# YuliangXiu/ICON

Measured on NVIDIA H100. Metric: M query-points/sec at 256^3 grid, higher is better.
Workload: dtype f32

## Files before the change

### icon_b200/csrc/common.cuh

```cuda
#pragma once
#include <cuda_runtime.h>
#include <stdint.h>
#include <stdio.h>

#include "../../include/icon_b200.h"

namespace icon {

void set_error(const char *fmt, ...);
void count_launch(int n = 1);

#define ICON_CHECK_ARG(cond, ...)                 \
    do {                                          \
        if (!(cond)) {                            \
            icon::set_error(__VA_ARGS__);         \
            return ICON_EINVAL;                   \
        }                                         \
    } while (0)

#define ICON_CUDA(expr)                                                              \
    do {                                                                             \
        cudaError_t _e = (expr);                                                     \
        if (_e != cudaSuccess) {                                                     \
            icon::set_error("%s:%d %s -> %s", __FILE__, __LINE__, #expr,             \
// ... 20 lines not shown
    return true;
}
int device_sm_count();

bool pdl_enabled();
#ifdef __CUDACC__
__device__ __forceinline__ void pdl_launch_dependents() { asm volatile("griddepcontrol.launch_dependents;" ::: "memory"); }
__device__ __forceinline__ void pdl_wait() { asm volatile("griddepcontrol.wait;" ::: "memory"); }
template <typename... KArgs, typename... Args>
static inline cudaError_t launch_pdl(void (*kernel)(KArgs...), dim3 grid, dim3 block, size_t smem, cudaStream_t stream,
                                     Args &&...args) {
    cudaLaunchConfig_t cfg = {};
    cfg.gridDim = grid; cfg.blockDim = block; cfg.dynamicSmemBytes = smem; cfg.stream = stream;
    cudaLaunchAttribute attr[1];
    attr[0].id = cudaLaunchAttributeProgrammaticStreamSerialization;
    attr[0].val.programmaticStreamSerializationAllowed = 1;
    cfg.attrs = attr; cfg.numAttrs = pdl_enabled() ? 1 : 0;
    return cudaLaunchKernelEx(&cfg, kernel, KArgs(args)...);
}

__device__ __forceinline__ void stats_add3(double *w, double s) {
    const double a = trunc(s), r = s - a;
    const double b = rint(r * 4294967296.0) * (1.0 / 4294967296.0);
    const double c = rint((r - b) * 18446744073709551616.0) * (1.0 / 18446744073709551616.0);
    if (a != 0.0) atomicAdd(w, a);
    if (b != 0.0) atomicAdd(w + 1, b);
    if (c != 0.0) atomicAdd(w + 2, c);
}
__device__ __forceinline__ void stats_add(double *st, double s1, double s2) { stats_add3(st, s1); stats_add3(st + 3, s2); }
__device__ __forceinline__ double stats_sum(const double *st) { return st[0] + (st[1] + st[2]); }
__device__ __forceinline__ double stats_sumsq(const double *st) { return st[3] + (st[4] + st[5]); }
#endif

struct Carver {
    char *base;
    size_t off;
    explicit Carver(void *p) : base((char *)p), off(0) {}
    template <typename T>
    T *take(size_t n) {
        off = align_up(off, 256);
        T *r = (T *)(base ? base + off : nullptr);
        off += n * sizeof(T);
        return r;
    }
    size_t total() const { return align_up(off, 256); }
};

constexpr int TREE_MAX_LEVELS = 17;
constexpr int RAY_GRID = 256;
constexpr int RAY_LIST_PER_FACE = 64;

constexpr int BRICK_AX = 32;
constexpr int NBRICK = BRICK_AX * BRICK_AX * BRICK_AX;
constexpr int BRICK_MAX_LEAVES = 4096;
constexpr int64_t BRICK_LIST_CAP = 1 << 24;
static inline int64_t brick_list_cap(int F) {
    const int64_t all = (int64_t)NBRICK * ((F + 3) / 4);
    return all < BRICK_LIST_CAP ? all : BRICK_LIST_CAP;
}

struct MeshHeader {
    float y0, z0, inv_cy, inv_cz;
    int ray_overflow;
    int brick_built;
    int brick_overflow;
    int pad;
};

struct FaceTree {
    float4 *tri_s;
    float4 *sph_s;
    int32_t *order;
    float4 *nodes;
    int F;
    int nlevels;
    int lvl_cnt[TREE_MAX_LEVELS];
    int lvl_off[TREE_MAX_LEVELS];
};

struct MeshView : FaceTree {
    const float4 *tri;
    const float4 *sph;
    const float4 *attr;
    const float4 *rbox;
    float *vnormals;
    unsigned long long *keys;
    int32_t *rcount;
    int32_t *roff;
    int32_t *rlist;
    MeshHeader *hdr;
    void *scan_ws;
    float4 *bxyz;
    int32_t *bperm;
    float *brec;
    int32_t *bface;
    float *bub;
    int32_t *boff;
    unsigned short *blist;
    int64_t brick_cap;
    int V;
};
size_t mesh_ws_bytes(int V, int F);
MeshView mesh_view(const void *ws, int V, int F);
void bricks_forget(const MeshView &m);

void profile_mark(int i, cudaStream_t stream);

size_t scan_ws_bytes(int64_t n);
int scan_exclusive_i32(const int32_t *in, int32_t *out, int64_t n, int64_t *d_total ,
                       void *ws, cudaStream_t stream);

}
```

### icon_b200/csrc/face_tree.cuh

```cuda
#pragma once
#include <float.h>

#include "common.cuh"
#include "geom.cuh"

namespace icon {

__device__ __forceinline__ float box_dist2(V3 p, float4 lo, float4 hi) {
    const float dx = fmaxf(fmaxf(lo.x - p.x, p.x - hi.x), 0.f);
    const float dy = fmaxf(fmaxf(lo.y - p.y, p.y - hi.y), 0.f);
    const float dz = fmaxf(fmaxf(lo.z - p.z, p.z - hi.z), 0.f);
    return fmaf(dz, dz, fmaf(dy, dy, dx * dx));
}
__device__ __forceinline__ float box_far2(V3 p, float4 lo, float4 hi) {
    const float dx = fmaxf(fabsf(lo.x - p.x), fabsf(hi.x - p.x));
    const float dy = fmaxf(fabsf(lo.y - p.y), fabsf(hi.y - p.y));
    const float dz = fmaxf(fabsf(lo.z - p.z), fabsf(hi.z - p.z));
    return fmaf(dz, dz, fmaf(dy, dy, dx * dx));
}
__device__ __forceinline__ float warp_max(float v) {
    for (int o = 16; o; o >>= 1) v = fmaxf(v, __shfl_xor_sync(0xffffffffu, v, o));
    return v;
}
__device__ __forceinline__ float warp_min(float v) {
// ... 38 lines not shown
    tri[2] = make_float4(ac.z, 0.f, 0.f, 0.f);
    *sph = make_float4(sc.x, sc.y, sc.z, sr);
    return sc;
}

__device__ __forceinline__ void write_leaf_box(const FaceTree &t, int n) {
    float4 lo = make_float4(FLT_MAX, FLT_MAX, FLT_MAX, 0.f), hi = make_float4(-FLT_MAX, -FLT_MAX, -FLT_MAX, 0.f);
    for (int k = 4 * n; k < min(4 * n + 4, t.F); ++k) {
        const Tri tr = load_tri(t.tri_s + 3 * (size_t)k);
        const V3 vs[3] = {tr.a, mk3(tr.a.x + tr.ab.x, tr.a.y + tr.ab.y, tr.a.z + tr.ab.z),
                          mk3(tr.a.x + tr.ac.x, tr.a.y + tr.ac.y, tr.a.z + tr.ac.z)};
        for (int j = 0; j < 3; ++j) {
            lo.x = fminf(lo.x, vs[j].x); hi.x = fmaxf(hi.x, vs[j].x);
            lo.y = fminf(lo.y, vs[j].y); hi.y = fmaxf(hi.y, vs[j].y);
            lo.z = fminf(lo.z, vs[j].z); hi.z = fmaxf(hi.z, vs[j].z);
        }
    }
    t.nodes[2 * (size_t)n] = lo;
    t.nodes[2 * (size_t)n + 1] = hi;
}

__device__ __forceinline__ void write_parent_box(const FaceTree &t, int l, int n) {
    const float4 *child = t.nodes + 2 * (size_t)t.lvl_off[l - 1];
    float4 lo = make_float4(FLT_MAX, FLT_MAX, FLT_MAX, 0.f), hi = make_float4(-FLT_MAX, -FLT_MAX, -FLT_MAX, 0.f);
    for (int c = 4 * n; c < min(4 * n + 4, t.lvl_cnt[l - 1]); ++c) {
        const float4 a = child[2 * (size_t)c], b = child[2 * (size_t)c + 1];
        lo.x = fminf(lo.x, a.x); lo.y = fminf(lo.y, a.y); lo.z = fminf(lo.z, a.z);
        hi.x = fmaxf(hi.x, b.x); hi.y = fmaxf(hi.y, b.y); hi.z = fmaxf(hi.z, b.z);
    }
    t.nodes[2 * ((size_t)t.lvl_off[l] + n)] = lo;
    t.nodes[2 * ((size_t)t.lvl_off[l] + n) + 1] = hi;
}

struct ChunkSmem {
    float4 sph[32];
    float4 tri[32][3];
    int kk[32];
};
template <typename Id, int CAP>
struct WalkSmem : ChunkSmem {
    Id fr[2][CAP];
};

template <int PPW>
struct NearestFace {
    static constexpr int REP = 32 / PPW;
    const int lane;
    V3 p;
    float tol, tol_sup;
    float best = FLT_MAX;
    int bi = 0x7fffffff;
    float sb = 0.f, ub = 0.f;
    int staged = 0;

    __device__ __forceinline__ NearestFace(V3 p_, float tol_, float tol_sup_)
        : lane(threadIdx.x & 31), p(p_), tol(tol_), tol_sup(tol_sup_) {}

    __device__ __forceinline__ float sphere_bound(float d) const {
        const float b = d * rsqrtf(d) * 1.00001f + tol;
        return d > 0.f ? b : tol;
    }

    __device__ __forceinline__ void try_face(const float4 *rec, int f) {
        const Tri tr = load_tri(rec);
        const float d = tri_sqdist(p, tr.a, tr.ab, tr.ac);
        if (d < best || (d == best && f < bi)) { best = d; bi = f; }
    }

    __device__ __forceinline__ void descend(const FaceTree &t, V3 c) {
        int node = 0;
        for (int lvl = t.nlevels - 1; lvl > 0; --lvl) {
            const int ch = 4 * node + (lane & 3);
            float a = FLT_MAX;
            int ai = ch;
            if (ch < t.lvl_cnt[lvl - 1]) {
                const float4 *nb = t.nodes + 2 * ((size_t)t.lvl_off[lvl - 1] + ch);
                a = box_dist2(c, __ldg(nb), __ldg(nb + 1));
            }
            for (int o = 1; o <= 2; o <<= 1) {
                const float ob = __shfl_xor_sync(0xffffffffu, a, o);
                const int oi = __shfl_xor_sync(0xffffffffu, ai, o);
                if (ob < a || (ob == a && oi < ai)) { a = ob; ai = oi; }
            }
            node = __shfl_sync(0xffffffffu, ai, 0);
        }
        for (int k = 4 * node; k < min(4 * node + 4, t.F); ++k) try_face(t.tri_s + 3 * (size_t)k, __ldg(t.order + k));
    }

    __device__ __forceinline__ void start_scan(float ubw) {
        sb = sphere_bound(best);
        ub = ubw * 1.00001f + tol;
    }

    __device__ __forceinline__ void test(const FaceTree &t, int k, float4 s, const float4 *tr) {
        const float dx = p.x - s.x, dy = p.y - s.y, dz = p.z - s.z;
        const float dd = fmaf(dz, dz, fmaf(dy, dy, dx * dx));
        const float l = sb + s.w;
        if (dd > l * l) return;
        const float4 r0 = tr[0], r1 = tr[1], r2 = tr[2];
        const V3 ab = mk3(r0.w, r1.x, r1.y), ac = mk3(r1.z, r1.w, r2.x);
        const float S1 = fmaf(dz, ab.z, fmaf(dy, ab.y, dx * ab.x));
        const float T1 = fmaf(dz, ac.z, fmaf(dy, ac.y, dx * ac.x));
        const float M = fmaxf(fmaxf(-(S1 + T1), fmaf(2.f, S1, -T1)), fmaf(2.f, T1, -S1)) * (1.f / 3.f);
        const float g = dd - M - tol_sup;
        if (g > 0.f && g * g > best * dd * 1.0001f) return;
        const float d = tri_sqdist(p, mk3(r0.x, r0.y, r0.z), ab, ac);
        if (!(d <= best)) return;
        const int f = __ldg(t.order + k);
        if (d < best || f < bi) { best = d; bi = f; sb = sphere_bound(d); }
    }

    __device__ __forceinline__ void merge() {
#pragma unroll
        for (int o = PPW; o < 32; o <<= 1) {
            const float ob = __shfl_xor_sync(0xffffffffu, best, o);
            const int oi = __shfl_xor_sync(0xffffffffu, bi, o);
            if (ob < best || (ob == best && oi < bi)) { best = ob; bi = oi; }
        }
    }

    __device__ __forceinline__ void chunk(const FaceTree &t, ChunkSmem &S, int leaf, float4 wlo, float4 whi) {
        bool pass = false;
        int k = 0;
        float4 s = make_float4(0.f, 0.f, 0.f, 0.f);
        if (leaf >= 0) {
            k = 4 * leaf + (lane & 3);
            if (k < t.F) {
                s = __ldg(t.sph_s + k);
                const float l2 = ub + s.w;
                pass = box_dist2(mk3(s.x, s.y, s.z), wlo, whi) <= l2 * l2;
            }
        }
        const unsigned mask = __ballot_sync(0xffffffffu, pass);
        const int cnt = __popc(mask);
        staged += cnt;
        if (pass) {
            const int at = __popc(mask & ((1u << lane) - 1u));
            const float4 *tp = t.tri_s + 3 * (size_t)k;
            S.sph[at] = s;
            S.kk[at] = k;
            S.tri[at][0] = __ldg(tp); S.tri[at][1] = __ldg(tp + 1); S.tri[at][2] = __ldg(tp + 2);
        }
        __syncwarp();
        for (int j = lane / PPW; j < cnt; j += REP) test(t, S.kk[j], S.sph[j], &S.tri[j][0]);
        if (REP > 1) {
            merge();
            sb = sphere_bound(best);
        }
        ub = fminf(ub, warp_max(sb));
        __syncwarp();
    }

    template <typename Id>
    __device__ __forceinline__ void scan_leaves(const FaceTree &t, ChunkSmem &S, const Id *leaves, int n, float4 wlo,
                                                float4 whi) {
        for (int base = 0; base < n; base += 8) {
            const int slot = base + (lane >> 2);
            chunk(t, S, slot < n ? (int)leaves[slot] : -1, wlo, whi);
// ... 68 lines not shown
```

### icon_b200/csrc/sdf.cu

```cuda
#include <float.h>

#include <algorithm>
#include <mutex>
#include <type_traits>
#include <unordered_set>

#include "common.cuh"
#include "face_tree.cuh"
#include "geom.cuh"

namespace icon {

struct Calib {
    float r[9];
    float t[3];
};

__device__ __forceinline__ V3 load_point(const float *__restrict__ pts, int64_t sc, int64_t sn,
                                         int64_t i, const Calib &cb) {
    float px = pts[i * sn], py = pts[sc + i * sn], pz = pts[2 * sc + i * sn];
    V3 o;
    o.x = fmaf(cb.r[2], pz, fmaf(cb.r[1], py, cb.r[0] * px)) + cb.t[0];
    o.y = fmaf(cb.r[5], pz, fmaf(cb.r[4], py, cb.r[3] * px)) + cb.t[1];
    o.z = fmaf(cb.r[8], pz, fmaf(cb.r[7], py, cb.r[6] * px)) + cb.t[2];
// ... 41 lines not shown
__device__ __forceinline__ unsigned spread7(unsigned v) {
    v = (v | (v << 16)) & 0x030000FFu;
    v = (v | (v << 8)) & 0x0300F00Fu;
    v = (v | (v << 4)) & 0x030C30C3u;
    v = (v | (v << 2)) & 0x09249249u;
    return v;
}

__device__ __forceinline__ int bin_of(V3 p) {
    const bool inside = p.x >= -1.f && p.x <= 1.f && p.y >= -1.f && p.y <= 1.f && p.z >= -1.f && p.z <= 1.f;
    if (!inside) return NBIN;
    const unsigned bx = min(NBIN_AX - 1, (int)((p.x + 1.f) * (NBIN_AX * 0.5f)));
    const unsigned by = min(NBIN_AX - 1, (int)((p.y + 1.f) * (NBIN_AX * 0.5f)));
    const unsigned bz = min(NBIN_AX - 1, (int)((p.z + 1.f) * (NBIN_AX * 0.5f)));
    return (int)(spread7(bx) | (spread7(by) << 1) | (spread7(bz) << 2));
}

__global__ void k_points_bin(const float *__restrict__ pts, int64_t sc, int64_t sn, int64_t N, Calib cb,
                             float4 *__restrict__ xyz4, int32_t *__restrict__ bid, int32_t *__restrict__ count) {
    const int64_t i = (int64_t)blockIdx.x * blockDim.x + threadIdx.x;
    const bool live = i < N;
    int b = -1;
    if (live) {
        const V3 p = load_point(pts, sc, sn, i, cb);
        const float in_cube = (p.x > -1.f && p.x < 1.f && p.y > -1.f && p.y < 1.f && p.z > -1.f && p.z < 1.f) ? 1.f : 0.f;
        xyz4[i] = make_float4(p.x, p.y, p.z, in_cube);
        b = bin_of(p);
        bid[i] = b;
    }
    const unsigned act = __ballot_sync(0xffffffffu, live);
    if (live) {
        const unsigned peers = __match_any_sync(act, b);
        if ((int)(threadIdx.x & 31) == __ffs(peers) - 1) atomicAdd(&count[b], __popc(peers));
    }
}

__global__ void k_points_scatter(const int32_t *__restrict__ bid, int64_t N, const int32_t *__restrict__ offset,
                                 int32_t *__restrict__ cursor, int32_t *__restrict__ perm) {
    const int64_t i = (int64_t)blockIdx.x * blockDim.x + threadIdx.x;
    const bool live = i < N;
    const int b = live ? bid[i] : -1;
    const unsigned act = __ballot_sync(0xffffffffu, live);
    if (live) {
        const unsigned peers = __match_any_sync(act, b);
        const int lane = threadIdx.x & 31, leader = __ffs(peers) - 1;
        int base = 0;
        if (lane == leader) base = atomicAdd(&cursor[b], __popc(peers));
        base = __shfl_sync(peers, base, leader);
        perm[offset[b] + base + __popc(peers & ((1u << lane) - 1u))] = (int32_t)i;
    }
}

#ifdef ICON_SDF_STATS
__device__ unsigned long long g_stats[8];
#define STAT(i, v) do { if (lane == 0) atomicAdd(&g_stats[i], (unsigned long long)(v)); } while (0)
#else
#define STAT(i, v) do { } while (0)
#endif

template <int PPW, bool BRICK>
using SdfSmem = typename std::conditional<BRICK, ChunkSmem, WalkSmem<unsigned short, fr_cap(PPW)>>::type;
template <int PPW, bool BRICK>
constexpr size_t sdf_smem_bytes() { return sizeof(SdfSmem<PPW, BRICK>) * (SW_T / 32); }

constexpr float BRICK_W = 2.0f / BRICK_AX;
constexpr float BRICK_HALF_DIAG = 0.0541266f;

__device__ __forceinline__ void brick_box(int b, float4 &lo, float4 &hi) {
    const int bx = b % BRICK_AX, by = (b / BRICK_AX) % BRICK_AX, bz = b / (BRICK_AX * BRICK_AX);
    lo = make_float4(-1.f + bx * BRICK_W, -1.f + by * BRICK_W, -1.f + bz * BRICK_W, 0.f);
    hi = make_float4(-1.f + (bx + 1) * BRICK_W, -1.f + (by + 1) * BRICK_W, -1.f + (bz + 1) * BRICK_W, 0.f);
}

__device__ __forceinline__ float leaf_key(const MeshView &m, int l, float4 lo, float4 hi) {
    const float4 a = __ldg(m.nodes + 2 * (size_t)l), z = __ldg(m.nodes + 2 * (size_t)l + 1);
    const float gx = fmaxf(fmaxf(a.x - hi.x, lo.x - z.x), 0.f);
    const float gy = fmaxf(fmaxf(a.y - hi.y, lo.y - z.y), 0.f);
    const float gz = fmaxf(fmaxf(a.z - hi.z, lo.z - z.z), 0.f);
    return fmaf(gz, gz, fmaf(gy, gy, gx * gx));
}

template <int PPW, bool BRICK>
__device__ __forceinline__ void sdf_warp(int64_t wid, SdfSmem<PPW, BRICK> &S, const float4 *__restrict__ xyz4,
                                         const int32_t *__restrict__ perm, int64_t N, const MeshView &m,
                                         float *__restrict__ rec, int32_t *__restrict__ face,
                                         int32_t *__restrict__ defer, int32_t *__restrict__ ndefer) {
    constexpr int REP = 32 / PPW;
    const int lane = threadIdx.x & 31;
    const int sub = lane % PPW, rep_id = lane / PPW;
    const int64_t pos0 = wid * PPW;
    const int64_t pos = pos0 + sub;
    if (pos0 >= N) return;
    const bool live = pos < N;
    const int64_t idx = perm[live ? pos : pos0];
    const float4 q = xyz4[idx];
    const V3 p = mk3(q.x, q.y, q.z);
    const V3 c = mk3(0.5f * (warp_min(p.x) + warp_max(p.x)), 0.5f * (warp_min(p.y) + warp_max(p.y)),
                     0.5f * (warp_min(p.z) + warp_max(p.z)));
    const float rw = warp_max(sqrtf(dot3(sub3(p, c), sub3(p, c)))) * 1.00001f + 1e-6f;
    const float4 wlo = make_float4(warp_min(p.x) - 1e-6f, warp_min(p.y) - 1e-6f, warp_min(p.z) - 1e-6f, 0.f);
    const float4 whi = make_float4(warp_max(p.x) + 1e-6f, warp_max(p.y) + 1e-6f, warp_max(p.z) + 1e-6f, 0.f);
    const MeshHeader h = *m.hdr;

    NearestFace<PPW> nf(p, 1e-6f, 1e-7f);
    if constexpr (BRICK) {
        bool ok = h.brick_built && !h.brick_overflow && c.x >= -1.f && c.x < 1.f && c.y >= -1.f && c.y < 1.f &&
                  c.z >= -1.f && c.z < 1.f;
        int b = 0;
        float4 blo, bhi;
        if (ok) {
            const int bx = min(BRICK_AX - 1, (int)((c.x + 1.f) * (BRICK_AX * 0.5f)));
            const int by = min(BRICK_AX - 1, (int)((c.y + 1.f) * (BRICK_AX * 0.5f)));
            const int bz = min(BRICK_AX - 1, (int)((c.z + 1.f) * (BRICK_AX * 0.5f)));
            b = (bz * BRICK_AX + by) * BRICK_AX + bx;
            brick_box(b, blo, bhi);
            ok = wlo.x >= blo.x && wlo.y >= blo.y && wlo.z >= blo.z && whi.x <= bhi.x && whi.y <= bhi.y && whi.z <= bhi.z;
        }
        if (!ok) {
            if (lane == 0) defer[atomicAdd(ndefer, 1)] = (int32_t)wid;
            return;
        }
        const int f = __ldg(m.bface + b);
        nf.try_face(m.tri + 3 * (size_t)f, f);
        nf.start_scan(fminf(warp_max(sqrtf(nf.best)), __ldg(m.bub + b)));
        STAT(0, 1);
        const int o1 = __ldg(m.boff + b + 1);
        for (int base = __ldg(m.boff + b); base < o1; base += 8) {
            const int slot = base + (lane >> 2);
            const int leaf = slot < o1 ? (int)__ldg(m.blist + slot) : -1;
            float key = 0.f;
            if (lane == 0) key = leaf_key(m, leaf, blo, bhi);
            if (__shfl_sync(0xffffffffu, key, 0) > nf.ub * nf.ub) break;
            STAT(2, min(8, o1 - base));
            nf.chunk(m, S, leaf, wlo, whi);
        }
        nf.merge();
    } else {
        const int n = tree_nearest(m, S, nf, c, rw, wlo, whi);
        STAT(0, 1); STAT(1, n > fr_cap(PPW) ? 1 : 0); STAT(2, n);
    }
    STAT(3, nf.staged);
    int hits = 0;
    if (!h.ray_overflow) {
        const float fy = (p.y - h.y0) * h.inv_cy, fz = (p.z - h.z0) * h.inv_cz;
        if (fy >= 0.f && fy < (float)RAY_GRID && fz >= 0.f && fz < (float)RAY_GRID) {
            const int cc = (int)fz * RAY_GRID + (int)fy;
            const int k0 = __ldg(m.roff + cc), k1 = __ldg(m.roff + cc + 1);
            for (int k = k0 + rep_id; k < k1; k += REP) {
                const int f = __ldg(m.rlist + k);
                if (__ldg(&m.rbox[2 * (size_t)f + 1].x) < p.x - 1e-3f) continue;
                const Tri tr = load_tri(m.tri + 3 * (size_t)f);
                hits += ray_hit_px(p, tr.a, tr.ab, tr.ac);
            }
        }
    } else {
        for (int f = rep_id; f < m.F; f += REP) {
            const Tri tr = load_tri(m.tri + 3 * (size_t)f);
            hits += ray_hit_px(p, tr.a, tr.ab, tr.ac);
        }
    }
    if (REP > 1) {
#pragma unroll
        for (int o = PPW; o < 32; o <<= 1) hits += __shfl_xor_sync(0xffffffffu, hits, o);
    }
    if (live && rep_id == 0) emit_record(p, nf.bi, nf.best, hits, m, rec, face, idx);
}

template <int PPW, bool BRICK>
__global__ void __launch_bounds__(SW_T) k_sdf_warp(const float4 *__restrict__ xyz4, const int32_t *__restrict__ perm,
                                                   int64_t N, MeshView m, float *__restrict__ rec,
                                                   int32_t *__restrict__ face, int32_t *__restrict__ defer,
                                                   int32_t *__restrict__ ndefer) {
    static_assert(!BRICK || PPW == 32, "brick lists serve dense lattices: 32 points per warp");
    extern __shared__ __align__(16) unsigned char smem_raw[];
    SdfSmem<PPW, BRICK> &S = reinterpret_cast<SdfSmem<PPW, BRICK> *>(smem_raw)[threadIdx.x >> 5];
    const bool listed = !BRICK && defer != nullptr;
    const int64_t nw = listed ? (int64_t)*ndefer : (N + PPW - 1) / PPW;
    for (int64_t i = (int64_t)blockIdx.x * (SW_T / 32) + (threadIdx.x >> 5); i < nw; i += (int64_t)gridDim.x * (SW_T / 32))
        sdf_warp<PPW, BRICK>(listed ? (int64_t)defer[i] : i, S, xyz4, perm, N, m, rec, face, defer, ndefer);
}

__global__ void k_brick_centres(MeshView m) {
    const int b = blockIdx.x * blockDim.x + threadIdx.x;
    if (b >= NBRICK) return;
    float4 lo, hi;
    brick_box(b, lo, hi);
    m.bxyz[b] = make_float4(0.5f * (lo.x + hi.x), 0.5f * (lo.y + hi.y), 0.5f * (lo.z + hi.z), 0.f);
    m.bperm[b] = b;
}

__global__ void __launch_bounds__(128) k_brick_count(MeshView m) {
    __shared__ int s_cnt;
    const int b = blockIdx.x;
    float4 lo, hi;
    brick_box(b, lo, hi);
    const float4 cc = m.bxyz[b];
    const Tri t = load_tri(m.tri + 3 * (size_t)m.bface[b]);
    const float d = tri_sqdist(mk3(cc.x, cc.y, cc.z), t.a, t.ab, t.ac);
    const float ub = (sqrtf(d) + BRICK_HALF_DIAG) * 1.00001f + 1e-6f, ub2 = ub * ub;
    if (threadIdx.x == 0) s_cnt = 0;
    __syncthreads();
    int cnt = 0;
    for (int l = threadIdx.x; l < m.lvl_cnt[0]; l += blockDim.x) cnt += leaf_key(m, l, lo, hi) <= ub2;
    for (int o = 16; o; o >>= 1) cnt += __shfl_xor_sync(0xffffffffu, cnt, o);
    if ((threadIdx.x & 31) == 0) atomicAdd(&s_cnt, cnt);
    __syncthreads();
    if (threadIdx.x == 0) {
        m.bub[b] = ub;
        m.boff[b] = s_cnt;
        if (s_cnt > BRICK_MAX_LEAVES) m.hdr->brick_overflow = 1;
        if (b == 0) m.boff[NBRICK] = 0;
    }
}

__global__ void __launch_bounds__(128) k_brick_fill(MeshView m, int64_t cap) {
    __shared__ float s_key[BRICK_MAX_LEAVES];
    __shared__ unsigned short s_leaf[BRICK_MAX_LEAVES];
    __shared__ int s_wcnt[4];
    if (m.hdr->brick_overflow || m.boff[NBRICK] > cap) return;
    const int b = blockIdx.x, o0 = m.boff[b], lane = threadIdx.x & 31, wib = threadIdx.x >> 5;
    float4 lo, hi;
    brick_box(b, lo, hi);
    const float ub = m.bub[b], ub2 = ub * ub;
    const int nleaf = m.lvl_cnt[0];
    int n = 0;
    for (int l0 = 0; l0 < nleaf; l0 += 128) {
        const int l = l0 + threadIdx.x;
        float key = 0.f;
        if (l < nleaf) key = leaf_key(m, l, lo, hi);
        const bool in = l < nleaf && key <= ub2;
        const unsigned bal = __ballot_sync(0xffffffffu, in);
        if (lane == 0) s_wcnt[wib] = __popc(bal);
        __syncthreads();
        int at = n + __popc(bal & ((1u << lane) - 1u));
        for (int w = 0; w < wib; ++w) at += s_wcnt[w];
        if (in) { s_key[at] = key; s_leaf[at] = (unsigned short)l; }
        n += s_wcnt[0] + s_wcnt[1] + s_wcnt[2] + s_wcnt[3];
        __syncthreads();
    }
    for (int i = threadIdx.x; i < n; i += blockDim.x) {
        const float k = s_key[i];
        int r = 0;
        for (int j = 0; j < n; ++j) {
            const float kj = s_key[j];
            r += kj < k || (kj == k && j < i);
        }
        m.blist[o0 + r] = s_leaf[i];
    }
}

__global__ void k_brick_done(MeshView m, int64_t cap) {
    if (m.boff[NBRICK] > cap) m.hdr->brick_overflow = 1;
    m.hdr->brick_built = 1;
}

__global__ void __launch_bounds__(256) k_sdf_brute(const float *__restrict__ pts, int64_t sc, int64_t sn,
                                                   int64_t N, Calib cb, MeshView m,
                                                   float *__restrict__ rec, int32_t *__restrict__ face) {
    __shared__ float4 tile[3 * 256];
    int64_t i = (int64_t)blockIdx.x * blockDim.x + threadIdx.x;
    bool live = i < N;
    V3 p = mk3(0.f, 0.f, 0.f);
    if (live) p = load_point(pts, sc, sn, i, cb);
    float best = FLT_MAX;
    int bi = 0, hits = 0;
    for (int f0 = 0; f0 < m.F; f0 += 256) {
        int nf = min(256, m.F - f0);
        __syncthreads();
        for (int k = threadIdx.x; k < 3 * nf; k += 256) tile[k] = m.tri[3 * (size_t)f0 + k];
        __syncthreads();
        if (live) {
            for (int k = 0; k < nf; ++k) {
                float4 r0 = tile[3 * k], r1 = tile[3 * k + 1], r2 = tile[3 * k + 2];
                V3 a = mk3(r0.x, r0.y, r0.z), ab = mk3(r0.w, r1.x, r1.y), ac = mk3(r1.z, r1.w, r2.x);
                float d = tri_sqdist(p, a, ab, ac);
                if (d < best) { best = d; bi = f0 + k; }
                hits += ray_hit_px(p, a, ab, ac);
            }
        }
    }
    if (live) emit_record(p, bi, best, hits, m, rec, face, i);
}

static int64_t g_sdf_ppw32_from = 6000000, g_sdf_ppw8_from = 300000;
static int g_sdf_ppw_force = 0;
static int g_sdf_bricks = 1;
static int64_t g_brick_max_entries = 0;

static std::mutex g_brick_mu;
static std::unordered_set<const void *> g_brick_ready;
static int64_t g_brick_builds = 0;

void bricks_forget(const MeshView &m) {
    std::lock_guard<std::mutex> lk(g_brick_mu);
    g_brick_ready.erase(m.hdr);
}

struct SdfWs {
    float4 *xyz4;
    int32_t *bid, *perm, *count, *offset;
    int32_t *defer, *ndefer;
    void *scan_ws;
};
static SdfWs carve_sdf(Carver &c, int64_t N) {
    SdfWs w;
    w.xyz4 = c.take<float4>((size_t)N);
    w.bid = c.take<int32_t>((size_t)N);
    w.perm = c.take<int32_t>((size_t)N);
    w.count = c.take<int32_t>(NBIN + 1);
    w.offset = c.take<int32_t>(NBIN + 1);
    w.defer = c.take<int32_t>((size_t)(N + 31) / 32);
    w.ndefer = c.take<int32_t>(1);
    w.scan_ws = c.take<char>(scan_ws_bytes(NBIN + 1));
    return w;
}

static int build_bricks(const MeshView &m, cudaStream_t stream) {
    const int64_t cap = g_brick_max_entries > 0 ? std::min(g_brick_max_entries, m.brick_cap) : m.brick_cap;
    k_brick_centres<<<NBRICK / 256, 256, 0, stream>>>(m);
    ICON_LAUNCHED();
    k_sdf_warp<1, false><<<NBRICK / (SW_T / 32), SW_T, sdf_smem_bytes<1, false>(), stream>>>(
        m.bxyz, m.bperm, NBRICK, m, m.brec, m.bface, nullptr, nullptr);
    ICON_LAUNCHED();
    k_brick_count<<<NBRICK, 128, 0, stream>>>(m);
    ICON_LAUNCHED();
    int rc = scan_exclusive_i32(m.boff, m.boff, NBRICK + 1, nullptr, m.scan_ws, stream);
    if (rc) return rc;
    k_brick_fill<<<NBRICK, 128, 0, stream>>>(m, cap);
    ICON_LAUNCHED();
    k_brick_done<<<1, 1, 0, stream>>>(m, cap);
    ICON_LAUNCHED();
    return ICON_OK;
}
size_t sdf_ws_bytes(int64_t N) {
    Carver c(nullptr);
    carve_sdf(c, N);
    return c.total();
}

Calib make_calib(const float *h) {
    Calib cb;
    for (int r = 0; r < 3; ++r) {
        for (int k = 0; k < 3; ++k) cb.r[3 * r + k] = h[4 * r + k];
        cb.t[r] = h[4 * r + 3];
    }
    return cb;
}

int run_sdf(const float *points, int64_t sc, int64_t sn, int64_t N, const float *h_calib,
            const MeshView &m, float *rec, int32_t *face, void *ws, float4 **xyz4_out,
            cudaStream_t stream) {
    Carver c(ws);
    SdfWs w = carve_sdf(c, N);
    Calib cb = make_calib(h_calib);
    profile_mark(0, stream);
    ICON_CUDA(cudaMemsetAsync(w.count, 0, sizeof(int32_t) * (NBIN + 1), stream));
    const unsigned nblk = (unsigned)((N + 255) / 256);
    k_points_bin<<<nblk, 256, 0, stream>>>(points, sc, sn, N, cb, w.xyz4, w.bid, w.count);
    ICON_LAUNCHED();
    int rc = scan_exclusive_i32(w.count, w.offset, NBIN + 1, nullptr, w.scan_ws, stream);
    if (rc) return rc;
    ICON_CUDA(cudaMemsetAsync(w.count, 0, sizeof(int32_t) * (NBIN + 1), stream));
    k_points_scatter<<<nblk, 256, 0, stream>>>(w.bid, N, w.offset, w.count, w.perm);
    ICON_LAUNCHED();
    static bool attr_set[ICON_MAX_DEVICES] = {};
    if (device_needs_setup(attr_set)) {
#define ICON_SDF_ATTR(P, B) ICON_CUDA(cudaFuncSetAttribute(k_sdf_warp<P, B>, cudaFuncAttributeMaxDynamicSharedMemorySize, \
                                                           (int)sdf_smem_bytes<P, B>()))
        ICON_SDF_ATTR(32, true); ICON_SDF_ATTR(32, false); ICON_SDF_ATTR(16, false); ICON_SDF_ATTR(8, false);
        ICON_SDF_ATTR(4, false); ICON_SDF_ATTR(2, false); ICON_SDF_ATTR(1, false);
#undef ICON_SDF_ATTR
    }
    profile_mark(1, stream);
    int ppw = N >= g_sdf_ppw32_from ? 32 : (N >= g_sdf_ppw8_from ? 8 : 1);
    if (g_sdf_ppw_force) ppw = g_sdf_ppw_force;
    const int wpb = SW_T / 32;
    const int64_t nwarps = (N + ppw - 1) / ppw;
    const unsigned nblk_w = (unsigned)((nwarps + wpb - 1) / wpb);
#define ICON_SDF_LAUNCH(P) k_sdf_warp<P, false><<<nblk_w, SW_T, sdf_smem_bytes<P, false>(), stream>>>( \
// ... 7 lines not shown
        if (build) {
            rc = build_bricks(m, stream);
            std::lock_guard<std::mutex> lk(g_brick_mu);
            if (rc) { g_brick_ready.erase(m.hdr); return rc; }
            ++g_brick_builds;
        }
        ICON_CUDA(cudaMemsetAsync(w.ndefer, 0, sizeof(int32_t), stream));
        k_sdf_warp<32, true><<<nblk_w, SW_T, sdf_smem_bytes<32, true>(), stream>>>(
            w.xyz4, w.perm, N, m, rec, face, w.defer, w.ndefer);
        ICON_LAUNCHED();
        const unsigned nblk_d = (unsigned)std::min<int64_t>(nblk_w, (int64_t)device_sm_count() * 16);
        k_sdf_warp<32, false><<<nblk_d, SW_T, sdf_smem_bytes<32, false>(), stream>>>(
            w.xyz4, w.perm, N, m, rec, face, w.defer, w.ndefer);
    } else {
        switch (ppw) {
            case 32: ICON_SDF_LAUNCH(32); break;
            case 16: ICON_SDF_LAUNCH(16); break;
            case 8: ICON_SDF_LAUNCH(8); break;
            case 4: ICON_SDF_LAUNCH(4); break;
            case 2: ICON_SDF_LAUNCH(2); break;
            default: ICON_SDF_LAUNCH(1); break;
        }
    }
#undef ICON_SDF_LAUNCH
    ICON_LAUNCHED();
    profile_mark(2, stream);
    if (xyz4_out) *xyz4_out = w.xyz4;
    return ICON_OK;
}

__global__ void k_points_only(const float *__restrict__ pts, int64_t sc, int64_t sn, int64_t N, Calib cb,
                              float4 *__restrict__ xyz4) {
    int64_t i = (int64_t)blockIdx.x * blockDim.x + threadIdx.x;
    if (i >= N) return;
    V3 p = load_point(pts, sc, sn, i, cb);
    float in_cube = (p.x > -1.f && p.x < 1.f && p.y > -1.f && p.y < 1.f && p.z > -1.f && p.z < 1.f) ? 1.f : 0.f;
    xyz4[i] = make_float4(p.x, p.y, p.z, in_cube);
}

int run_points_only(const float *points, int64_t sc, int64_t sn, int64_t N, const float *h_calib,
                    float4 *xyz4, cudaStream_t stream) {
    Calib cb = make_calib(h_calib);
    k_points_only<<<(unsigned)((N + 255) / 256), 256, 0, stream>>>(points, sc, sn, N, cb, xyz4);
    ICON_LAUNCHED();
    return ICON_OK;
}

}

using namespace icon;

#ifdef ICON_SDF_STATS
extern "C" int icon_debug_sdf_stats(unsigned long long *out, int reset) {
    cudaMemcpyFromSymbol(out, icon::g_stats, sizeof(unsigned long long) * 8);
    if (reset) { unsigned long long z[8] = {0}; cudaMemcpyToSymbol(icon::g_stats, z, sizeof(z)); }
    return 0;
}
#endif

extern "C" int icon_set_sdf_policy(int force_ppw, int64_t ppw8_from, int64_t ppw32_from) {
    ICON_CHECK_ARG(force_ppw >= 0 && force_ppw <= 32 && (force_ppw & (force_ppw - 1)) == 0, "icon_set_sdf_policy: ppw in {0,1,2,4,8,16,32}");
    icon::g_sdf_ppw_force = force_ppw;
    if (ppw8_from >= 0) icon::g_sdf_ppw8_from = ppw8_from;
    if (ppw32_from >= 0) icon::g_sdf_ppw32_from = ppw32_from;
    return ICON_OK;
}

extern "C" int icon_set_sdf_bricks(int enable, int64_t max_entries) {
    ICON_CHECK_ARG(enable == 0 || enable == 1, "icon_set_sdf_bricks: enable must be 0 or 1");
    icon::g_sdf_bricks = enable;
    icon::g_brick_max_entries = max_entries > 0 ? max_entries : 0;
    return ICON_OK;
}

extern "C" int icon_sdf_brick_info(const void *mesh_ws, int V, int F, int64_t *out) {
    ICON_CHECK_ARG(mesh_ws && out && V > 0 && F > 0, "icon_sdf_brick_info: bad argument");
    MeshView m = mesh_view(mesh_ws, V, F);
    MeshHeader h;
    int32_t total = 0;
    ICON_CUDA(cudaDeviceSynchronize());
    ICON_CUDA(cudaMemcpy(&h, m.hdr, sizeof(h), cudaMemcpyDeviceToHost));
    if (h.brick_built) ICON_CUDA(cudaMemcpy(&total, m.boff + NBRICK, sizeof(total), cudaMemcpyDeviceToHost));
    out[0] = h.brick_built;
    out[1] = h.brick_overflow;
    out[2] = total;
    out[3] = m.brick_cap;
    {
        std::lock_guard<std::mutex> lk(icon::g_brick_mu);
        out[4] = icon::g_brick_builds;
    }
    return ICON_OK;
}

extern "C" int icon_sdf_only(const float *points, int64_t stride_c, int64_t stride_n, int64_t N,
                             const float *h_calib, const void *mesh_ws, int V, int F, float *rec,
                             int32_t *face, void *ws, size_t ws_bytes, icon_stream_t stream_) {
    cudaStream_t stream = (cudaStream_t)stream_;
    ICON_CHECK_ARG(N >= 0 && N < (int64_t)INT32_MAX, "icon_sdf_only: N=%lld out of range", (long long)N);
    if (N == 0) return ICON_OK;
    ICON_CHECK_ARG(points && h_calib && mesh_ws && rec && ws, "icon_sdf_only: null pointer");
    if (ws_bytes < sdf_ws_bytes(N)) {
        set_error("icon_sdf_only: workspace %zu < %zu", ws_bytes, sdf_ws_bytes(N));
        return ICON_ENOSPC;
    }
    MeshView m = mesh_view(mesh_ws, V, F);
    return run_sdf(points, stride_c, stride_n, N, h_calib, m, rec, face, ws, nullptr, stream);
}

extern "C" int icon_sdf_bruteforce(const float *points, int64_t stride_c, int64_t stride_n, int64_t N,
                                   const float *h_calib, const void *mesh_ws, int V, int F, float *rec,
                                   int32_t *face, icon_stream_t stream_) {
    cudaStream_t stream = (cudaStream_t)stream_;
    if (N == 0) return ICON_OK;
    ICON_CHECK_ARG(points && h_calib && mesh_ws && rec, "icon_sdf_bruteforce: null pointer");
    MeshView m = mesh_view(mesh_ws, V, F);
    Calib cb = make_calib(h_calib);
    k_sdf_brute<<<(unsigned)((N + 255) / 256), 256, 0, stream>>>(points, stride_c, stride_n, N, cb, m, rec, face);
    ICON_LAUNCHED();
    return ICON_OK;
}
```

### icon_b200/csrc/smpl.cu

```cuda
#include <float.h>

#include "common.cuh"
#include "face_tree.cuh"
#include "geom.cuh"

namespace icon {

static MeshView carve_mesh(Carver &c, int V, int F) {
    MeshView m{};
    m.V = V;
    const size_t total_nodes = tree_levels(m, F);
    m.tri = c.take<float4>((size_t)F * 3);
    m.sph = c.take<float4>((size_t)F);
    m.attr = c.take<float4>((size_t)F * 6);
    m.rbox = c.take<float4>((size_t)F * 2);
    m.keys = c.take<unsigned long long>((size_t)F);
    m.order = c.take<int32_t>((size_t)F);
    m.tri_s = c.take<float4>((size_t)F * 3);
    m.sph_s = c.take<float4>((size_t)F);
    m.nodes = c.take<float4>(total_nodes * 2);
    m.rcount = c.take<int32_t>(RAY_GRID * RAY_GRID + 1);
    m.roff = c.take<int32_t>(RAY_GRID * RAY_GRID + 1);
    m.rlist = c.take<int32_t>((size_t)F * RAY_LIST_PER_FACE);
    m.hdr = c.take<MeshHeader>(1);
    m.scan_ws = c.take<char>(scan_ws_bytes(RAY_GRID * RAY_GRID + 1));
    m.bxyz = c.take<float4>(NBRICK);
    m.bperm = c.take<int32_t>(NBRICK);
    m.brec = c.take<float>((size_t)NBRICK * 8);
    m.bface = c.take<int32_t>(NBRICK);
    m.bub = c.take<float>(NBRICK);
    m.boff = c.take<int32_t>(NBRICK + 1);
    m.brick_cap = brick_list_cap(F);
    m.blist = c.take<unsigned short>((size_t)m.brick_cap);
    m.vnormals = c.take<float>((size_t)V * 3);
    return m;
}

size_t mesh_ws_bytes(int V, int F) {
    Carver c(nullptr);
    carve_mesh(c, V, F);
    return c.total();
}

MeshView mesh_view(const void *ws, int V, int F) {
    Carver c((void *)ws);
    return carve_mesh(c, V, F);
}

__global__ void __launch_bounds__(128) k_vertex_normals(const float *__restrict__ verts,
                                                        const int64_t *__restrict__ faces, int V, int F,
                                                        float *__restrict__ out) {
    __shared__ int s_faces[3 * 512];
    const int v = blockIdx.x * blockDim.x + threadIdx.x;
    float sx = 0.f, sy = 0.f, sz = 0.f;
    for (int pass = 0; pass < 3; ++pass) {
        const int corner = (pass == 0) ? 1 : (pass == 1 ? 2 : 0);
        const int c1 = (corner + 1) % 3, c2 = (corner + 2) % 3;
        for (int f0 = 0; f0 < F; f0 += 512) {
            const int nf = min(512, F - f0);
            __syncthreads();
            for (int k = threadIdx.x; k < 3 * nf; k += blockDim.x) s_faces[k] = (int)faces[3 * (size_t)f0 + k];
            __syncthreads();
            if (v < V) {
                for (int k = 0; k < nf; ++k) {
                    if (s_faces[3 * k + corner] != v) continue;
                    const int i1 = s_faces[3 * k + c1], i2 = s_faces[3 * k + c2];
                    V3 p0 = mk3(verts[3 * v], verts[3 * v + 1], verts[3 * v + 2]);
                    V3 p1 = mk3(verts[3 * i1], verts[3 * i1 + 1], verts[3 * i1 + 2]);
                    V3 p2 = mk3(verts[3 * i2], verts[3 * i2 + 1], verts[3 * i2 + 2]);
                    V3 n = cross3(sub3(p1, p0), sub3(p2, p0));
                    sx += n.x; sy += n.y; sz += n.z;
                }
            }
        }
    }
    if (v >= V) return;
    float nrm = sqrtf(sx * sx + sy * sy + sz * sz);
    if (nrm < 1e-6f) nrm = 1e-6f;
    out[3 * v] = sx / nrm;
    out[3 * v + 1] = sy / nrm;
    out[3 * v + 2] = sz / nrm;
}

__global__ void k_face_records(const float *__restrict__ verts, const int64_t *__restrict__ faces,
                               const float *__restrict__ vnormals, const float *__restrict__ cmap,
                               const float *__restrict__ vis, int F, float4 *__restrict__ tri,
// ... 150 lines not shown
```

Baseline: 556.6.

## Refine SDF brick candidate lists to 64^3 sub-bricks

Splits each 32^3 brick into eight sub-bricks and builds a separate sorted leaf candidate list for each one. Each sub-brick gets its own tighter upper bound from its centre, so a query point scans fewer leaves. Parent-brick leaves are gathered once and then filtered per sub-brick. The brick scratch buffers now alias the list storage to save memory. The cost is a larger build (8x centre SDFs, bigger lists) and a higher chance of overflowing the list cap.

```diff
diff --git a/icon_b200/csrc/common.cuh b/icon_b200/csrc/common.cuh
--- a/icon_b200/csrc/common.cuh
+++ b/icon_b200/csrc/common.cuh
@@ -96,10 +96,12 @@
 
 constexpr int BRICK_AX = 32;
 constexpr int NBRICK = BRICK_AX * BRICK_AX * BRICK_AX;
+constexpr int SUB_AX = 2 * BRICK_AX;
+constexpr int NSUB = SUB_AX * SUB_AX * SUB_AX;
 constexpr int BRICK_MAX_LEAVES = 4096;
-constexpr int64_t BRICK_LIST_CAP = 1 << 24;
+constexpr int64_t BRICK_LIST_CAP = 40 << 20;
 static inline int64_t brick_list_cap(int F) {
-    const int64_t all = (int64_t)NBRICK * ((F + 3) / 4);
+    const int64_t all = (int64_t)NSUB * ((F + 3) / 4);
     return all < BRICK_LIST_CAP ? all : BRICK_LIST_CAP;
 }
 
@@ -134,13 +136,13 @@
     int32_t *rlist;
     MeshHeader *hdr;
     void *scan_ws;
-    float4 *bxyz;
-    int32_t *bperm;
-    float *brec;
     int32_t *bface;
     float *bub;
     int32_t *boff;
     unsigned short *blist;
+    float4 *bxyz;
+    int32_t *bperm;
+    float *brec;
     int64_t brick_cap;
     int V;
 };
diff --git a/icon_b200/csrc/face_tree.cuh b/icon_b200/csrc/face_tree.cuh
--- a/icon_b200/csrc/face_tree.cuh
+++ b/icon_b200/csrc/face_tree.cuh
@@ -114,6 +114,7 @@
     int bi = 0x7fffffff;
     float sb = 0.f, ub = 0.f;
     int staged = 0;
+    int exact = 0;
 
     __device__ __forceinline__ NearestFace(V3 p_, float tol_, float tol_sup_)
         : lane(threadIdx.x & 31), p(p_), tol(tol_), tol_sup(tol_sup_) {}
@@ -166,6 +167,7 @@
         const float M = fmaxf(fmaxf(-(S1 + T1), fmaf(2.f, S1, -T1)), fmaf(2.f, T1, -S1)) * (1.f / 3.f);
         const float g = dd - M - tol_sup;
         if (g > 0.f && g * g > best * dd * 1.0001f) return;
+        ++exact;
         const float d = tri_sqdist(p, mk3(r0.x, r0.y, r0.z), ab, ac);
         if (!(d <= best)) return;
         const int f = __ldg(t.order + k);
diff --git a/icon_b200/csrc/sdf.cu b/icon_b200/csrc/sdf.cu
--- a/icon_b200/csrc/sdf.cu
+++ b/icon_b200/csrc/sdf.cu
@@ -117,10 +117,13 @@
 }
 
 #ifdef ICON_SDF_STATS
-__device__ unsigned long long g_stats[8];
-#define STAT(i, v) do { if (lane == 0) atomicAdd(&g_stats[i], (unsigned long long)(v)); } while (0)
+constexpr int SDF_NSTATS = 16;
+__device__ unsigned long long g_stats[SDF_NSTATS];
+#define STAT(i, v) do { if (lane == 0) atomicAdd(&g_stats[(BRICK ? 0 : 8) + (i)], (unsigned long long)(v)); } while (0)
+#define STAT_LANES(i, v) do { atomicAdd(&g_stats[(BRICK ? 0 : 8) + (i)], (unsigned long long)(v)); } while (0)
 #else
 #define STAT(i, v) do { } while (0)
+#define STAT_LANES(i, v) do { } while (0)
 #endif
 
 template <int PPW, bool BRICK>
@@ -128,13 +131,19 @@
 template <int PPW, bool BRICK>
 constexpr size_t sdf_smem_bytes() { return sizeof(SdfSmem<PPW, BRICK>) * (SW_T / 32); }
 
-constexpr float BRICK_W = 2.0f / BRICK_AX;
-constexpr float BRICK_HALF_DIAG = 0.0541266f;
-
-__device__ __forceinline__ void brick_box(int b, float4 &lo, float4 &hi) {
+constexpr float SUB_HALF_DIAG = 0.0271f;
+
+template <int AX>
+__device__ __forceinline__ void grid_box(int b, float4 &lo, float4 &hi) {
+    constexpr float W = 2.0f / AX;
+    const int bx = b % AX, by = (b / AX) % AX, bz = b / (AX * AX);
+    lo = make_float4(-1.f + bx * W, -1.f + by * W, -1.f + bz * W, 0.f);
+    hi = make_float4(-1.f + (bx + 1) * W, -1.f + (by + 1) * W, -1.f + (bz + 1) * W, 0.f);
+}
+
+__device__ __forceinline__ int sub_of(int b, int j) {
     const int bx = b % BRICK_AX, by = (b / BRICK_AX) % BRICK_AX, bz = b / (BRICK_AX * BRICK_AX);
-    lo = make_float4(-1.f + bx * BRICK_W, -1.f + by * BRICK_W, -1.f + bz * BRICK_W, 0.f);
-    hi = make_float4(-1.f + (bx + 1) * BRICK_W, -1.f + (by + 1) * BRICK_W, -1.f + (bz + 1) * BRICK_W, 0.f);
+    return ((2 * bz + (j >> 2)) * SUB_AX + 2 * by + ((j >> 1) & 1)) * SUB_AX + 2 * bx + (j & 1);
 }
 
 __device__ __forceinline__ float leaf_key(const MeshView &m, int l, float4 lo, float4 hi) {
@@ -174,14 +183,15 @@
         int b = 0;
         float4 blo, bhi;
         if (ok) {
-            const int bx = min(BRICK_AX - 1, (int)((c.x + 1.f) * (BRICK_AX * 0.5f)));
-            const int by = min(BRICK_AX - 1, (int)((c.y + 1.f) * (BRICK_AX * 0.5f)));
-            const int bz = min(BRICK_AX - 1, (int)((c.z + 1.f) * (BRICK_AX * 0.5f)));
-            b = (bz * BRICK_AX + by) * BRICK_AX + bx;
-            brick_box(b, blo, bhi);
+            const int bx = min(SUB_AX - 1, (int)((c.x + 1.f) * (SUB_AX * 0.5f)));
+            const int by = min(SUB_AX - 1, (int)((c.y + 1.f) * (SUB_AX * 0.5f)));
+            const int bz = min(SUB_AX - 1, (int)((c.z + 1.f) * (SUB_AX * 0.5f)));
+            b = (bz * SUB_AX + by) * SUB_AX + bx;
+            grid_box<SUB_AX>(b, blo, bhi);
             ok = wlo.x >= blo.x && wlo.y >= blo.y && wlo.z >= blo.z && whi.x <= bhi.x && whi.y <= bhi.y && whi.z <= bhi.z;
         }
         if (!ok) {
+            STAT(1, 1);
             if (lane == 0) defer[atomicAdd(ndefer, 1)] = (int32_t)wid;
             return;
         }
@@ -205,6 +215,7 @@
         STAT(0, 1); STAT(1, n > fr_cap(PPW) ? 1 : 0); STAT(2, n);
     }
     STAT(3, nf.staged);
+    STAT_LANES(4, nf.exact);
     int hits = 0;
     if (!h.ray_overflow) {
         const float fy = (p.y - h.y0) * h.inv_cy, fz = (p.z - h.z0) * h.inv_cz;
@@ -216,6 +227,7 @@
                 if (__ldg(&m.rbox[2 * (size_t)f + 1].x) < p.x - 1e-3f) continue;
                 const Tri tr = load_tri(m.tri + 3 * (size_t)f);
                 hits += ray_hit_px(p, tr.a, tr.ab, tr.ac);
+                STAT_LANES(5, 1);
             }
         }
     } else {
@@ -246,76 +258,118 @@
 }
 
 __global__ void k_brick_centres(MeshView m) {
-    const int b = blockIdx.x * blockDim.x + threadIdx.x;
-    if (b >= NBRICK) return;
+    const int s = blockIdx.x * blockDim.x + threadIdx.x;
+    if (s >= NSUB) return;
     float4 lo, hi;
-    brick_box(b, lo, hi);
-    m.bxyz[b] = make_float4(0.5f * (lo.x + hi.x), 0.5f * (lo.y + hi.y), 0.5f * (lo.z + hi.z), 0.f);
-    m.bperm[b] = b;
-}
-
-__global__ void __launch_bounds__(128) k_brick_count(MeshView m) {
-    __shared__ int s_cnt;
-    const int b = blockIdx.x;
+    grid_box<SUB_AX>(s, lo, hi);
+    m.bxyz[s] = make_float4(0.5f * (lo.x + hi.x), 0.5f * (lo.y + hi.y), 0.5f * (lo.z + hi.z), 0.f);
+    m.bperm[s] = s;
+}
+
+__device__ __forceinline__ int compact_slot(bool in, int &n, int *s_wcnt) {
+    const int lane = threadIdx.x & 31, wib = threadIdx.x >> 5;
+    const unsigned bal = __ballot_sync(0xffffffffu, in);
+    if (lane == 0) s_wcnt[wib] = __popc(bal);
+    __syncthreads();
+    int at = n + __popc(bal & ((1u << lane) - 1u));
+    for (int w = 0; w < wib; ++w) at += s_wcnt[w];
+    n += s_wcnt[0] + s_wcnt[1] + s_wcnt[2] + s_wcnt[3];
+    __syncthreads();
+    return at;
+}
+
+__device__ int parent_leaves(const MeshView &m, int b, const float *s_ub, unsigned short *s_leaf, int *s_wcnt) {
+    float ub = s_ub[0];
+    for (int j = 1; j < 8; ++j) ub = fmaxf(ub, s_ub[j]);
+    const float ub2 = ub * ub;
     float4 lo, hi;
-    brick_box(b, lo, hi);
-    const float4 cc = m.bxyz[b];
-    const Tri t = load_tri(m.tri + 3 * (size_t)m.bface[b]);
-    const float d = tri_sqdist(mk3(cc.x, cc.y, cc.z), t.a, t.ab, t.ac);
-    const float ub = (sqrtf(d) + BRICK_HALF_DIAG) * 1.00001f + 1e-6f, ub2 = ub * ub;
-    if (threadIdx.x == 0) s_cnt = 0;
-    __syncthreads();
-    int cnt = 0;
-    for (int l = threadIdx.x; l < m.lvl_cnt[0]; l += blockDim.x) cnt += leaf_key(m, l, lo, hi) <= ub2;
-    for (int o = 16; o; o >>= 1) cnt += __shfl_xor_sync(0xffffffffu, cnt, o);
-    if ((threadIdx.x & 31) == 0) atomicAdd(&s_cnt, cnt);
-    __syncthreads();
-    if (threadIdx.x == 0) {
-        m.bub[b] = ub;
-        m.boff[b] = s_cnt;
-        if (s_cnt > BRICK_MAX_LEAVES) m.hdr->brick_overflow = 1;
-        if (b == 0) m.boff[NBRICK] = 0;
-    }
-}
-
-__global__ void __launch_bounds__(128) k_brick_fill(MeshView m, int64_t cap) {
-    __shared__ float s_key[BRICK_MAX_LEAVES];
-    __shared__ unsigned short s_leaf[BRICK_MAX_LEAVES];
-    __shared__ int s_wcnt[4];
-    if (m.hdr->brick_overflow || m.boff[NBRICK] > cap) return;
-    const int b = blockIdx.x, o0 = m.boff[b], lane = threadIdx.x & 31, wib = threadIdx.x >> 5;
-    float4 lo, hi;
-    brick_box(b, lo, hi);
-    const float ub = m.bub[b], ub2 = ub * ub;
+    grid_box<BRICK_AX>(b, lo, hi);
     const int nleaf = m.lvl_cnt[0];
     int n = 0;
     for (int l0 = 0; l0 < nleaf; l0 += 128) {
         const int l = l0 + threadIdx.x;
-        float key = 0.f;
-        if (l < nleaf) key = leaf_key(m, l, lo, hi);
-        const bool in = l < nleaf && key <= ub2;
-        const unsigned bal = __ballot_sync(0xffffffffu, in);
-        if (lane == 0) s_wcnt[wib] = __popc(bal);
+        const bool in = l < nleaf && leaf_key(m, l, lo, hi) <= ub2;
+        const int at = compact_slot(in, n, s_wcnt);
+        if (in && at < BRICK_MAX_LEAVES) s_leaf[at] = (unsigned short)l;
+    }
+    __syncthreads();
+    return n;
+}
+
+__global__ void __launch_bounds__(128) k_brick_count(MeshView m) {
+    __shared__ unsigned short s_leaf[BRICK_MAX_LEAVES];
+    __shared__ float s_ub[8];
+    __shared__ int s_cnt[8], s_wcnt[4];
+    const int b = blockIdx.x;
+    if (threadIdx.x < 8) {
+        const int s = sub_of(b, threadIdx.x);
+        const float4 cc = m.bxyz[s];
+        const Tri t = load_tri(m.tri + 3 * (size_t)m.bface[s]);
+        const float d = tri_sqdist(mk3(cc.x, cc.y, cc.z), t.a, t.ab, t.ac);
+        const float ub = (sqrtf(d) + SUB_HALF_DIAG) * 1.00001f + 1e-6f;
+        s_ub[threadIdx.x] = ub;
+        m.bub[s] = ub;
+        s_cnt[threadIdx.x] = 0;
+    }
+    __syncthreads();
+    const int np = parent_leaves(m, b, s_ub, s_leaf, s_wcnt);
+    if (np > BRICK_MAX_LEAVES && threadIdx.x == 0) m.hdr->brick_overflow = 1;
+    const int nk = min(np, BRICK_MAX_LEAVES);
+    for (int j = 0; j < 8; ++j) {
+        float4 lo, hi;
+        grid_box<SUB_AX>(sub_of(b, j), lo, hi);
+        const float ub2 = s_ub[j] * s_ub[j];
+        int cnt = 0;
+        for (int i = threadIdx.x; i < nk; i += 128) cnt += leaf_key(m, s_leaf[i], lo, hi) <= ub2;
+        for (int o = 16; o; o >>= 1) cnt += __shfl_xor_sync(0xffffffffu, cnt, o);
+        if ((threadIdx.x & 31) == 0) atomicAdd(&s_cnt[j], cnt);
+    }
+    __syncthreads();
+    if (threadIdx.x < 8) m.boff[sub_of(b, threadIdx.x)] = s_cnt[threadIdx.x];
+    if (b == 0 && threadIdx.x == 0) m.boff[NSUB] = 0;
+}
+
+__global__ void __launch_bounds__(128) k_brick_fill(MeshView m, int64_t cap) {
+    __shared__ unsigned short s_leaf[BRICK_MAX_LEAVES], s_sub[BRICK_MAX_LEAVES];
+    __shared__ float s_key[BRICK_MAX_LEAVES];
+    __shared__ float s_ub[8];
+    __shared__ int s_wcnt[4];
+    if (m.hdr->brick_overflow || m.boff[NSUB] > cap) return;
+    const int b = blockIdx.x;
+    if (threadIdx.x < 8) s_ub[threadIdx.x] = m.bub[sub_of(b, threadIdx.x)];
+    __syncthreads();
+    const int np = parent_leaves(m, b, s_ub, s_leaf, s_wcnt);
+    for (int j = 0; j < 8; ++j) {
+        const int s = sub_of(b, j), o0 = m.boff[s];
+        float4 lo, hi;
+        grid_box<SUB_AX>(s, lo, hi);
+        const float ub2 = s_ub[j] * s_ub[j];
+        int n = 0;
+        for (int i0 = 0; i0 < np; i0 += 128) {
+            const int i = i0 + threadIdx.x;
+            int l = 0;
+            float key = 0.f;
+            if (i < np) { l = s_leaf[i]; key = leaf_key(m, l, lo, hi); }
+            const bool in = i < np && key <= ub2;
+            const int at = compact_slot(in, n, s_wcnt);
+            if (in) { s_key[at] = key; s_sub[at] = (unsigned short)l; }
+        }
         __syncthreads();
-        int at = n + __popc(bal & ((1u << lane) - 1u));
-        for (int w = 0; w < wib; ++w) at += s_wcnt[w];
-        if (in) { s_key[at] = key; s_leaf[at] = (unsigned short)l; }
-        n += s_wcnt[0] + s_wcnt[1] + s_wcnt[2] + s_wcnt[3];
+        for (int i = threadIdx.x; i < n; i += 128) {
+            const float k = s_key[i];
+            int r = 0;
+            for (int q = 0; q < n; ++q) {
+                const float kq = s_key[q];
+                r += kq < k || (kq == k && q < i);
+            }
+            m.blist[o0 + r] = s_sub[i];
+        }
         __syncthreads();
     }
-    for (int i = threadIdx.x; i < n; i += blockDim.x) {
-        const float k = s_key[i];
-        int r = 0;
-        for (int j = 0; j < n; ++j) {
-            const float kj = s_key[j];
-            r += kj < k || (kj == k && j < i);
-        }
-        m.blist[o0 + r] = s_leaf[i];
-    }
 }
 
 __global__ void k_brick_done(MeshView m, int64_t cap) {
-    if (m.boff[NBRICK] > cap) m.hdr->brick_overflow = 1;
+    if (m.boff[NSUB] > cap) m.hdr->brick_overflow = 1;
     m.hdr->brick_built = 1;
 }
 
@@ -382,14 +436,14 @@
 
 static int build_bricks(const MeshView &m, cudaStream_t stream) {
     const int64_t cap = g_brick_max_entries > 0 ? std::min(g_brick_max_entries, m.brick_cap) : m.brick_cap;
-    k_brick_centres<<<NBRICK / 256, 256, 0, stream>>>(m);
-    ICON_LAUNCHED();
-    k_sdf_warp<1, false><<<NBRICK / (SW_T / 32), SW_T, sdf_smem_bytes<1, false>(), stream>>>(
-        m.bxyz, m.bperm, NBRICK, m, m.brec, m.bface, nullptr, nullptr);
+    k_brick_centres<<<NSUB / 256, 256, 0, stream>>>(m);
+    ICON_LAUNCHED();
+    k_sdf_warp<1, false><<<NSUB / (SW_T / 32), SW_T, sdf_smem_bytes<1, false>(), stream>>>(
+        m.bxyz, m.bperm, NSUB, m, m.brec, m.bface, nullptr, nullptr);
     ICON_LAUNCHED();
     k_brick_count<<<NBRICK, 128, 0, stream>>>(m);
     ICON_LAUNCHED();
-    int rc = scan_exclusive_i32(m.boff, m.boff, NBRICK + 1, nullptr, m.scan_ws, stream);
+    int rc = scan_exclusive_i32(m.boff, m.boff, NSUB + 1, nullptr, m.scan_ws, stream);
     if (rc) return rc;
     k_brick_fill<<<NBRICK, 128, 0, stream>>>(m, cap);
     ICON_LAUNCHED();
@@ -503,8 +557,8 @@
 
 #ifdef ICON_SDF_STATS
 extern "C" int icon_debug_sdf_stats(unsigned long long *out, int reset) {
-    cudaMemcpyFromSymbol(out, icon::g_stats, sizeof(unsigned long long) * 8);
-    if (reset) { unsigned long long z[8] = {0}; cudaMemcpyToSymbol(icon::g_stats, z, sizeof(z)); }
+    cudaMemcpyFromSymbol(out, icon::g_stats, sizeof(unsigned long long) * icon::SDF_NSTATS);
+    if (reset) { unsigned long long z[icon::SDF_NSTATS] = {0}; cudaMemcpyToSymbol(icon::g_stats, z, sizeof(z)); }
     return 0;
 }
 #endif
@@ -531,7 +585,7 @@
     int32_t total = 0;
     ICON_CUDA(cudaDeviceSynchronize());
     ICON_CUDA(cudaMemcpy(&h, m.hdr, sizeof(h), cudaMemcpyDeviceToHost));
-    if (h.brick_built) ICON_CUDA(cudaMemcpy(&total, m.boff + NBRICK, sizeof(total), cudaMemcpyDeviceToHost));
+    if (h.brick_built) ICON_CUDA(cudaMemcpy(&total, m.boff + NSUB, sizeof(total), cudaMemcpyDeviceToHost));
     out[0] = h.brick_built;
     out[1] = h.brick_overflow;
     out[2] = total;
diff --git a/icon_b200/csrc/smpl.cu b/icon_b200/csrc/smpl.cu
--- a/icon_b200/csrc/smpl.cu
+++ b/icon_b200/csrc/smpl.cu
@@ -23,15 +23,24 @@
     m.roff = c.take<int32_t>(RAY_GRID * RAY_GRID + 1);
     m.rlist = c.take<int32_t>((size_t)F * RAY_LIST_PER_FACE);
     m.hdr = c.take<MeshHeader>(1);
-    m.scan_ws = c.take<char>(scan_ws_bytes(RAY_GRID * RAY_GRID + 1));
-    m.bxyz = c.take<float4>(NBRICK);
-    m.bperm = c.take<int32_t>(NBRICK);
-    m.brec = c.take<float>((size_t)NBRICK * 8);
-    m.bface = c.take<int32_t>(NBRICK);
-    m.bub = c.take<float>(NBRICK);
-    m.boff = c.take<int32_t>(NBRICK + 1);
+    m.scan_ws = c.take<char>(scan_ws_bytes((RAY_GRID * RAY_GRID > NSUB ? RAY_GRID * RAY_GRID : NSUB) + 1));
+    m.bface = c.take<int32_t>(NSUB);
+    m.bub = c.take<float>(NSUB);
+    m.boff = c.take<int32_t>(NSUB + 1);
     m.brick_cap = brick_list_cap(F);
-    m.blist = c.take<unsigned short>((size_t)m.brick_cap);
+    {
+        Carver s(nullptr);
+        s.take<float4>(NSUB);
+        s.take<int32_t>(NSUB);
+        s.take<float>((size_t)NSUB * 8);
+        const size_t list_bytes = sizeof(unsigned short) * (size_t)m.brick_cap;
+        char *lists = c.take<char>(list_bytes > s.total() ? list_bytes : s.total());
+        Carver b(lists);
+        m.bxyz = b.take<float4>(NSUB);
+        m.bperm = b.take<int32_t>(NSUB);
+        m.brec = b.take<float>((size_t)NSUB * 8);
+        m.blist = (unsigned short *)lists;
+    }
     m.vnormals = c.take<float>((size_t)V * 3);
     return m;
 }
```

After: 561.2 (median of 6 runs). About the same (+0.8%).
